# VinAIResearch/COMBAT

Hardware: AMD Instinct MI355X
Metric: images/sec per alternated generator+surrogate step, CIFAR-10 bs=128, 1/2/4/8 GPU (higher is better)
Workload: dtype bf16; 1 GPU; train_generator.py --dataset cifar10 --pc 0.5 --noise_rate 0.08: alternated PreActResNet18 surrogate + UNet generator step (Phase C + Phase G, both Nesterov-SGD updates), bs=128 per GPU, on-device augmentation on; per_gpu_batch=128, global_batch=128, parallelism=dp1 (RCCL all-reduce of netC grads in Phase C, netG grads in Phase G), losses_finite=True, deterministic=True

## Files before the change

### combat_amd/_lib.py

```python
from __future__ import annotations

import ctypes as C
import os

HERE = os.path.dirname(os.path.abspath(__file__))
LIB_PATH = os.environ.get("COMBAT_HIP_LIB") or os.path.join(HERE, "libcombat_hip.so")

c_i32, c_i64, c_f32, c_vp = C.c_int32, C.c_int64, C.c_float, C.c_void_p


class ConvArgs(C.Structure):

    _fields_ = [
        ("N", c_i32), ("H", c_i32), ("W", c_i32), ("C", c_i32),
        ("P", c_i32), ("Q", c_i32), ("K", c_i32),
        ("R", c_i32), ("S", c_i32), ("stride", c_i32), ("pad", c_i32),
        ("mode", c_i32),
        ("src", c_vp), ("wpack", c_vp), ("kpad", c_i32), ("rows_pad", c_i32), ("dst", c_vp),
        ("pro_scale", c_vp), ("pro_shift", c_vp), ("pro_group_stride", c_i32), ("pro_act", c_i32),
        ("pro_slope", c_f32),
        ("bias", c_vp), ("add_pre", c_vp), ("mask_x", c_vp), ("mask_scale", c_vp), ("mask_shift", c_vp),
        ("mask_activated", c_i32), ("mask_group_stride", c_i32), ("mask_slope", c_f32), ("mask_mul_scale", c_i32),
        ("add_post", c_vp), ("tanh_out", c_i32),
        ("stats_kind", c_i32), ("stats", c_vp), ("xh_mean", c_vp), ("xh_rstd", c_vp),
# ... 36 lines not shown

SIGNATURES = {
    "combat_version": (C.c_char_p, []),
    "combat_abi_version": (C.c_int, []),
    "combat_set_deterministic": (None, [C.c_int]),
    "combat_get_deterministic": (C.c_int, []),
    "combat_conv_gemm": (C.c_int, [C.POINTER(ConvArgs), c_vp]),
    "combat_conv_gemm_pair": (C.c_int, [C.POINTER(ConvArgs), C.POINTER(ConvArgs), c_vp]),
    "combat_conv_workspace_bytes": (c_i64, [C.POINTER(ConvArgs)]),
    "combat_conv_pick_tile": (C.c_int, [C.POINTER(ConvArgs)]),
    "combat_conv_stats_granule": (C.c_int, [C.c_int]),
    "combat_conv_stats_layout": (C.c_int, [C.POINTER(ConvArgs), C.POINTER(c_i32), C.POINTER(c_i32)]),
    "combat_conv_wgrad": (C.c_int, [C.POINTER(WgradArgs), c_vp]),
    "combat_conv_wgrad_workspace_bytes": (c_i64, [C.POINTER(WgradArgs)]),
    "combat_conv_wgrad_reduce": (C.c_int, [C.POINTER(WgradArgs), c_vp]),
    "combat_pack_weights": (C.c_int, [c_vp, c_i32, c_i32, c_i32, c_i32, c_i32, c_vp, c_i32, c_i32, c_vp, c_i32,
                                      c_i32, c_vp]),
    "combat_norm_finalize": (C.c_int, [c_vp, c_i32, c_i32, c_i32, c_f32, c_f32, c_vp, c_vp, c_vp, c_vp, c_vp, c_vp,
                                       c_vp, c_vp, c_f32, c_vp, c_vp, c_i64, c_vp]),
    "combat_norm_scratch_bytes": (c_i64, [c_i32, c_i32]),
    "combat_bn_eval_fold": (C.c_int, [c_vp, c_vp, c_vp, c_vp, c_f32, c_i32, c_vp, c_vp, c_vp]),
    "combat_pack_weights_batch": (C.c_int, [c_vp, c_i32, c_vp]),
    "combat_bn_eval_fold_batch": (C.c_int, [c_vp, c_i32, c_f32, c_vp]),
    "combat_group_stats": (C.c_int, [c_vp, c_i32, c_i32, c_i32, c_vp, c_vp]),
    "combat_norm_bwd_finalize": (C.c_int, [c_vp, c_i32, c_i32, c_i32, c_f32, c_vp, c_vp, c_vp, c_vp, c_vp, c_vp,
                                           c_vp, c_vp, c_vp, c_i64, c_vp]),
    "combat_norm_bwd_apply": (C.c_int, [c_vp, c_vp, c_vp, c_vp, c_i64, c_i32, c_i32, c_i32, c_vp, c_vp, c_vp, c_vp]),
    "combat_norm_act_fused": (C.c_int, [c_vp, c_vp, c_i32, c_i32, c_i64, c_i32, c_f32, c_f32, c_vp, c_vp, c_vp, c_vp, c_vp,
                                        c_vp, c_vp, c_vp, c_f32, c_vp, c_vp, c_i64, c_vp, c_vp]),
    "combat_norm_add_act_fused": (C.c_int, [c_vp, c_vp, c_i32, c_i32, c_i64, c_i32, c_f32, c_f32, c_vp, c_vp, c_vp, c_vp, c_vp,
# ... 114 lines not shown
```

### combat_amd/csrc/capi.cpp

```cpp
#include "combat_hip.h"

#include <hip/hip_runtime.h>

#include <atomic>
#include <cstdlib>
#include <mutex>
#include <unordered_map>

#define COMBAT_ABI_VERSION 20

extern "C" const char *combat_version(void) { return "combat_hip gfx950 abi17"; }
extern "C" int combat_abi_version(void) { return COMBAT_ABI_VERSION; }

static std::atomic<int> g_deterministic{-1};
bool combat_deterministic() {
    int v = g_deterministic.load(std::memory_order_relaxed);
    if (v < 0) {
        const char *e = getenv("COMBAT_DETERMINISTIC");
        v = e && e[0] == '1';
        g_deterministic.store(v, std::memory_order_relaxed);
    }
    return v != 0;
}
extern "C" void combat_set_deterministic(int on) { g_deterministic.store(on ? 1 : 0, std::memory_order_relaxed); }
// ... 19 lines not shown
```

### combat_amd/csrc/conv_common.hpp

```cpp
#pragma once
#include "common.hpp"
#include <type_traits>

int conv3x3_pick(const combat_conv_args *a);
int conv3x3_stats_layout(const combat_conv_args *a, int tile, int *rows, int *rows_per_image);
int conv3x3_launch(const combat_conv_args *a, int tile, hipStream_t st);
int conv3x3d_pick(const combat_conv_args *a);
int conv3x3d_stats_layout(const combat_conv_args *a, int tile, int *rows, int *rows_per_image);
int conv3x3d_launch(const combat_conv_args *a, int tile, hipStream_t st);
int conv_gather_dma_bn(const combat_conv_args *a);
bool conv_gather_dma_parity_split(const combat_conv_args *a);
bool conv_c8_ok(const combat_conv_args *a);
int conv_c8_launch(const combat_conv_args *a, hipStream_t st);
bool conv_k8_ok(const combat_conv_args *a);
int conv_k8_launch(const combat_conv_args *a, hipStream_t st);
int conv_gather_dma_launch(const combat_conv_args *a, hipStream_t st);
int conv_gather_dma_pair_launch(const combat_conv_args *a, const combat_conv_args *b, hipStream_t st);
long conv_gather_dma_workspace(const combat_conv_args *a);
int conv_wgrad3x3_try(const combat_wgrad_args *a, hipStream_t st);
int conv_wgrad3x3_dma_try(const combat_wgrad_args *a, hipStream_t st);
long conv_wgrad3x3_dma_workspace(const combat_wgrad_args *a);
int conv_wgrad3x3_dma_reduce(const combat_wgrad_args *a, hipStream_t st);

template <int BM, int BN, int WGM_ = 0>
struct TileCfg {
    static constexpr int WGM = WGM_ ? WGM_ : ((BN == 16) ? 4 : 2);
    static constexpr int WGN = 4 / WGM;
    static constexpr int WM = BM / WGM;
    static constexpr int WN = BN / WGN;
    static constexpr int FM = WM / 16;
    static constexpr int FN = WN / 16;
    static constexpr int A_ITERS = BM / 32;
    static constexpr int B_ITERS = (BN + 31) / 32;
    static constexpr int EPS = BN + 4;
    static constexpr int STAGE_BYTES = 2 * (BM + BN) * 128;
    static constexpr int EP_BYTES = BM * EPS * 4;
    static constexpr int SMEM = STAGE_BYTES > EP_BYTES ? STAGE_BYTES : EP_BYTES;
// ... 181 lines not shown
```

### combat_amd/csrc/conv_wgrad.hip

```cpp
#include "conv_common.hpp"
#include "plan.hpp"

namespace {

struct WgradParams {
    combat_wgrad_args a;
    int M, PQ, ntaps, tiles_k, tiles_c, split, pix_per_split;
    float *ws;
};

template <int BMC, int BNC>
struct WCfg {
    static constexpr int WGK = (BNC == 16) ? 4 : (BMC == 16 ? 1 : 2);
    static constexpr int WGC = 4 / WGK;
    static constexpr int WK = BMC / WGK;
    static constexpr int WC = BNC / WGC;
    static constexpr int FK = WK / 16;
    static constexpr int FC = WC / 16;
    static constexpr int SK = (BMC + 16) * 2;
    static constexpr int SC = (BNC + 16) * 2;
    static constexpr int CHK = BMC / 8;
    static constexpr int CHC = BNC / 8;
    static constexpr int ITK = (64 * CHK + 255) / 256;
    static constexpr int ITC = (64 * CHC + 255) / 256;
// ... 550 lines not shown
    if (a->R != a->S || (a->R != 1 && a->R != 3)) return COMBAT_EINVAL;
    if (a->stride != 1 && a->stride != 2) return COMBAT_EINVAL;
    if (a->c_real <= 0 || a->c_real > a->C || a->k_real <= 0 || a->k_real > a->K) return COMBAT_EINVAL;
    if ((a->pro_scale == nullptr) != (a->pro_shift == nullptr)) return COMBAT_EINVAL;
    if ((long)a->N * a->P * a->Q > 0x7fffffffL / 8) return COMBAT_EINVAL;
    return COMBAT_OK;
}

extern "C" int combat_conv_wgrad_reduce(const combat_wgrad_args *a, void *stream) {
    COMBAT_PLAN_HOOK(combat_conv_wgrad_reduce, a);
    if (validate_wgrad_args(a) != COMBAT_OK) return COMBAT_EINVAL;
    if (a->split < 0 || !a->defer_reduce) return COMBAT_OK;
    return conv_wgrad3x3_dma_reduce(a, as_stream(stream));
}

extern "C" int combat_conv_wgrad(const combat_wgrad_args *a, void *stream) {
    COMBAT_PLAN_HOOK(combat_conv_wgrad, a);
    if (validate_wgrad_args(a) != COMBAT_OK) return COMBAT_EINVAL;
    WgradParams p;
    p.a = *a;
    p.ws = nullptr;
    p.PQ = a->P * a->Q;
    p.M = (int)((long)a->N * p.PQ);
    p.ntaps = a->R * a->S;
    hipStream_t st = as_stream(stream);
    if (a->split >= 0) {
        int rc = conv_wgrad3x3_dma_try(a, st);
        if (rc <= 0) return rc;
    }
    if (a->reduce_first) {
// ... 15 lines not shown
```

### combat_amd/csrc/conv_wgrad3x3_dma.hip

```cpp
#include "conv_common.hpp"
#include <stdlib.h>

namespace {

typedef __attribute__((address_space(3))) void lds_void_t;
constexpr unsigned kOob = 0x40000000u;

struct W3dParams {
    combat_wgrad_args a;
    int TW, TH, TI, HWP, HH, HROWS, hpw, tw_shift, th_shift;
    int tiles_x, tiles_y, ntiles, tiles_k, tiles_c, split, per;
    unsigned x_bytes, dy_bytes;
    float *ws;
    const float *red_ws;
    float *red_dw;
    int red_base, red_tiles_c, red_split, red_k_real, red_c_real, red_pad;
    unsigned long long *stamps;
};

#ifdef COMBAT_STAMPS
static unsigned long long *g_stamps_wgrad_host = nullptr;
extern "C" int combat_debug_set_stamps_wgrad(void *p) { g_stamps_wgrad_host = (unsigned long long *)p; return 0; }
#define WCLK() __builtin_readcyclecounter()
#else
// ... 78 lines not shown
                const int row = (i * 2 + (wave & 1)) * 16 + (lane >> 4) * 4, col = (wave >> 1) * 16 + (lane & 15);
                const int tile_c = tile % tiles_c, tile_k = tile / tiles_c;
                const int n = tile_k * 64 + row, c = tile_c * 64 + col;
                if (c < c_real) {
#pragma unroll
                    for (int e = 0; e < 4; ++e)
                        if (n + e < k_real) dw[((size_t)(n + e) * 9 + tap) * c_real + c] += acc[u][e];
                }
            }
        }
        if (SL > 1) __syncthreads();
    }
}

template <int HPW, int NS, bool RED>
__device__ __forceinline__ void wgrad3x3_dma_body(const W3dParams &p) {
    extern __shared__ __attribute__((aligned(16))) unsigned char smem[];
    const combat_wgrad_args &a = p.a;
    const int tid = threadIdx.x, lane = tid & 63;
    const int wid = __builtin_amdgcn_readfirstlane(tid >> 6);
    const int wave_k = wid & 1, wave_c = wid >> 1;
    if (RED && p.red_ws) {
        reduce_slabs<512>(p.red_ws, p.red_dw, p.red_base, p.red_tiles_c, p.red_split, p.red_k_real, p.red_c_real, smem, blockIdx.x, gridDim.x);
        __syncthreads();
    }
    int bid = blockIdx.x;
    const int tile_c = bid % p.tiles_c; bid /= p.tiles_c;
    const int tile_k = bid % p.tiles_k;
    const int sp = bid / p.tiles_k;
    const int k0 = tile_k * 64, c0 = tile_c * 64;
    const int t_begin = sp * p.per;
    int t_end = t_begin + p.per;
    if (t_end > p.ntiles) t_end = p.ntiles;
    if (t_begin >= t_end) return;

    const int C = a.C, K = a.K, H = a.H, W = a.W;
    constexpr int XBYTES = HPW * 8192, DYBYTES = 64 * 128, DYBASE = NS * XBYTES;
    constexpr int NDMA = 1 + HPW;
    auto rsrc_words = [&](const void *ptr, unsigned bytes) __attribute__((always_inline)) {
        const unsigned long base = (unsigned long)ptr;
        u32x4_t w;
        w[0] = __builtin_amdgcn_readfirstlane((unsigned)base);
        w[1] = __builtin_amdgcn_readfirstlane((unsigned)(base >> 32) & 0xffffu);
        w[2] = __builtin_amdgcn_readfirstlane(bytes);
        w[3] = 0x00020000u;
        return w;
    };
    const u32x4_t xrs = rsrc_words(a.src, p.x_bytes), dyrs = rsrc_words(a.dy, p.dy_bytes);
    const unsigned lds0 = __builtin_amdgcn_readfirstlane((unsigned)(unsigned long)(lds_void_t *)smem) + wid * 1024;
#ifdef COMBAT_WGRAD_BUILTIN_DMA
    const __amdgpu_buffer_rsrc_t xrsrc = __builtin_amdgcn_make_buffer_rsrc(const_cast<void *>(a.src), 0, p.x_bytes, 0x00020000);
    const __amdgpu_buffer_rsrc_t dyrsrc = __builtin_amdgcn_make_buffer_rsrc(const_cast<void *>(a.dy), 0, p.dy_bytes, 0x00020000);
#define COMBAT_W3_DMA(rs_builtin, rs_words, lds_off, voff) \
    __builtin_amdgcn_raw_ptr_buffer_load_lds(rs_builtin, (lds_void_t *)(smem + (lds_off) + wid * 1024), 16, voff, 0, 0, 0)
#else
#define COMBAT_W3_DMA(rs_builtin, rs_words, lds_off, voff) \
    asm volatile("s_mov_b32 m0, %0\n\ts_nop 0\n\tbuffer_load_dwordx4 %1, %2, 0 offen lds" ::"s"(lds0_l + (unsigned)(lds_off)), "v"(voff), "s"(rs_words##_l) : "memory", "m0")
#endif

    int hdec[HPW], hrel[HPW];
#pragma unroll
    for (int j = 0; j < HPW; ++j) {
        const int row = (wid + 8 * j) * 8 + (lane >> 3), slot = lane & 7;
        const int hx = row % p.HWP, line = row / p.HWP;
        const int hy = line % p.HH, ti = line / p.HH;
        const int chunk = (((slot >> 1) ^ xkey(p.TW, line, hx)) << 1) | (slot & 1);
        hdec[j] = row < p.HROWS ? (hx | (hy << 8) | (ti << 16)) : -1;
// ... 172 lines not shown
#else
        (void)c0; (void)c1; (void)c2;
#endif
    };
    for (int i = 0; i < npatch; i += NS) {
        body(integral_constant<int, 0>{}, i);
        if (NS > 1 && i + 1 < npatch) body(integral_constant<int, 1 % NS>{}, i + 1);
        if (NS > 2 && i + 2 < npatch) body(integral_constant<int, 2 % NS>{}, i + 2);
    }
    }
    static_assert(NS == 2 || NS == 3, "the patch loop is unrolled for rings of two or three stages");
#ifdef COMBAT_STAMPS
    const unsigned long long c_loop1 = WCLK();
#endif

    if (p.ws) {
        float *slab = p.ws + (size_t)blockIdx.x * 9 * 4096;
#pragma unroll
        for (int tap = 0; tap < 9; ++tap)
#pragma unroll
            for (int i = 0; i < 2; ++i)
                *reinterpret_cast<f32x4_t *>(slab + tap * 4096 + ((i * 8 + wid) * 64 + lane) * 4) = acc[tap][i];
    } else {
        float *ep = reinterpret_cast<float *>(smem);
        constexpr int EPS = 68;
        const int fr = lane & 15;
#pragma unroll 1
        for (int tap = 0; tap < 9; ++tap) {
#pragma unroll
            for (int i = 0; i < 2; ++i) {
                const int col = wave_c * 16 + fr;
                const int row = (i * 2 + wave_k) * 16 + fq * 4;
// ... 4 lines not shown
                    case 2: v = acc[2][i]; break;
                    case 3: v = acc[3][i]; break;
                    case 4: v = acc[4][i]; break;
                    case 5: v = acc[5][i]; break;
                    case 6: v = acc[6][i]; break;
                    case 7: v = acc[7][i]; break;
                    default: v = acc[8][i]; break;
                }
#pragma unroll
                for (int e = 0; e < 4; ++e) ep[(row + e) * EPS + col] = v[e];
            }
            __syncthreads();
            for (int idx = tid; idx < 64 * 64; idx += 512) {
                const int row = idx >> 6, col = idx & 63;
                const int n = k0 + row, c = c0 + col;
                if (n < a.k_real && c < a.c_real) atomicAdd(a.dw + ((size_t)n * 9 + tap) * a.c_real + c, ep[row * EPS + col]);
            }
            __syncthreads();
        }
    }
#ifdef COMBAT_STAMPS
    if (lane == 0 && p.stamps) {
        unsigned long long *o = p.stamps + (blockIdx.x * 8 + wid) * 8;
        o[0] = ph[0]; o[1] = ph[1]; o[2] = ph[2]; o[3] = ph[3];
        o[4] = c_loop1 - c_loop0; o[5] = WCLK() - c_loop1; o[6] = c_loop0;
    }
#endif
}

__global__ __launch_bounds__(256) void wgrad3x3_reduce_kernel(const float *__restrict__ ws, float *__restrict__ dw,
                                                              int base, int tiles_c, int split, int k_real, int c_real) {
    const long e4 = (long)blockIdx.x * 256 + threadIdx.x;
    if (e4 >= (long)base * 9 * 1024) return;
    const int f4 = (int)(e4 & 1023), tap = (int)((e4 >> 10) % 9), tile = (int)(e4 / (9 * 1024));
    const int per = (split + gridDim.y - 1) / gridDim.y;
    const int s0 = blockIdx.y * per, s1 = s0 + per < split ? s0 + per : split;
    f32x4_t acc = {0.f, 0.f, 0.f, 0.f};
    const float *src = ws + ((size_t)tile * 9 + tap) * 4096 + f4 * 4;
    const size_t sstride = (size_t)base * 9 * 4096;
    int s = s0;
    for (; s + 4 <= s1; s += 4) {
        const f32x4_t v0 = *reinterpret_cast<const f32x4_t *>(src + (size_t)s * sstride);
        const f32x4_t v1 = *reinterpret_cast<const f32x4_t *>(src + (size_t)(s + 1) * sstride);
        const f32x4_t v2 = *reinterpret_cast<const f32x4_t *>(src + (size_t)(s + 2) * sstride);
        const f32x4_t v3 = *reinterpret_cast<const f32x4_t *>(src + (size_t)(s + 3) * sstride);
        acc += (v0 + v1) + (v2 + v3);
// ... 2 lines not shown
    const int i = f4 >> 9, wave = (f4 >> 6) & 7, lane = f4 & 63;
    const int row = (i * 2 + (wave & 1)) * 16 + (lane >> 4) * 4, col = (wave >> 1) * 16 + (lane & 15);
    const int tile_c = tile % tiles_c, tile_k = tile / tiles_c;
    const int n = tile_k * 64 + row, c = tile_c * 64 + col;
    if (c < c_real && s0 < s1) {
#pragma unroll
        for (int e = 0; e < 4; ++e) {
            if (n + e >= k_real) break;
            float *o = dw + ((size_t)(n + e) * 9 + tap) * c_real + c;
            if (gridDim.y == 1) *o += acc[e];
            else atomicAdd(o, acc[e]);
        }
    }
}

__global__ __launch_bounds__(256) void wgrad3x3_reduce_det_kernel(const float *__restrict__ ws, float *__restrict__ dw, int base,
                                                                  int tiles_c, int split, int k_real, int c_real) {
    __shared__ __attribute__((aligned(16))) unsigned char scratch[256 * 64];
    reduce_slabs<256>(ws, dw, base, tiles_c, split, k_real, c_real, scratch, blockIdx.x, gridDim.x);
}

template <int HPW, int NS, bool RED>
__global__ __launch_bounds__(512, 1) void conv_wgrad3x3_dma_kernel(const W3dParams p) { wgrad3x3_dma_body<HPW, NS, RED>(p); }

template <int HPW, int NS, bool RED>
int launch_w3d_red(const W3dParams &p, int blocks, hipStream_t st) {
    constexpr int stage = 8192 + HPW * 8192;
    constexpr int ep = 64 * 68 * 4;
    constexpr int smem = NS * stage > ep ? NS * stage : ep;
    auto kern = conv_wgrad3x3_dma_kernel<HPW, NS, RED>;
    static bool attr = false;
    if (!attr) {
        if (hipFuncSetAttribute(reinterpret_cast<const void *>(kern), hipFuncAttributeMaxDynamicSharedMemorySize, smem) != hipSuccess)
            return COMBAT_ELAUNCH;
        attr = true;
    }
    COMBAT_LAUNCH(kern, dim3(blocks), dim3(512), smem, st, p);
    CB_LAUNCH_CHECK();
    return COMBAT_OK;
}

template <int HPW, int NS>
int launch_w3d(const W3dParams &p, int blocks, hipStream_t st) {
    return p.red_ws ? launch_w3d_red<HPW, NS, true>(p, blocks, st) : launch_w3d_red<HPW, NS, false>(p, blocks, st);
}

bool w3d_geometry(const combat_wgrad_args *a, W3dParams &p, int &smem) {
    if (!(a->R == 3 && a->S == 3 && a->stride == 1 && a->pad == 1 && a->P == a->H && a->Q == a->W)) return false;
    if (a->pro_scale || a->pro_act) return false;
    if (a->C < 64 || (a->C & 63) || a->K < 64 || (a->K & 63) || a->c_real != a->C) return false;
    const int W = a->W, H = a->H;
    const int TW = W < 16 ? W : 16;
// ... 45 lines not shown

namespace {
bool w3d_plan(const combat_wgrad_args *a, W3dParams &p) {
    int smem;
    if (!w3d_geometry(a, p, smem)) return false;
    const int base = p.tiles_k * p.tiles_c;
    int split = pick_split(a, p, true);
    const bool use_ws = split > 1 && a->workspace && a->workspace_bytes >= (long)split * base * 9 * 4096 * 4;
    if (!use_ws) split = pick_split(a, p, false);
    p.ws = use_ws ? reinterpret_cast<float *>(a->workspace) : nullptr;
    p.per = (p.ntiles + split - 1) / split;
    p.split = (p.ntiles + p.per - 1) / p.per;
    return true;
}

int launch_reduce(const combat_wgrad_args *a, const W3dParams &p, hipStream_t st) {
    const int base = p.tiles_k * p.tiles_c;
    static const bool env_det = getenv("COMBAT_WGRAD_DET_REDUCE") != nullptr;
    const bool det = combat_deterministic();
    const bool atomics = !env_det && (!det || base >= 4);
    if (atomics) {
        const long e4 = (long)base * 9 * 1024;
        int groups = (int)(512 / ((e4 + 255) / 256));
        if (groups < 1 || det) groups = 1;
        if (groups > p.split) groups = p.split;
        COMBAT_LAUNCH(wgrad3x3_reduce_kernel, dim3((unsigned)((e4 + 255) / 256), groups), dim3(256), 0, st, p.ws, a->dw, base,
                           p.tiles_c, p.split, a->k_real, a->c_real);
    } else {
        COMBAT_LAUNCH(wgrad3x3_reduce_det_kernel, dim3(256), dim3(256), 0, st, (const float *)p.ws, a->dw, base, p.tiles_c, p.split,
                           a->k_real, a->c_real);
    }
    CB_LAUNCH_CHECK();
    return COMBAT_OK;
}

bool fill_reduce_first(const combat_wgrad_args *prev, W3dParams &p) {
    p.red_ws = nullptr;
    p.red_dw = nullptr;
    p.red_base = p.red_tiles_c = p.red_split = p.red_k_real = p.red_c_real = p.red_pad = 0;
    if (!prev) return true;
    W3dParams q;
    if (!w3d_plan(prev, q)) return true;
// ... 21 lines not shown
#endif
    const int blocks = p.tiles_k * p.tiles_c * p.split;
    int rc;
    if (p.hpw == 2) rc = launch_w3d<2, 3>(p, blocks, st);
    else if (p.hpw == 3) rc = launch_w3d<3, 2>(p, blocks, st);
    else rc = launch_w3d<4, 2>(p, blocks, st);
    if (rc != COMBAT_OK || !p.ws || a->defer_reduce) return rc;
    return launch_reduce(a, p, st);
}

int conv_wgrad3x3_dma_reduce(const combat_wgrad_args *a, hipStream_t st) {
    W3dParams p;
    if (!w3d_plan(a, p) || !p.ws) return COMBAT_OK;
    return launch_reduce(a, p, st);
}
```

### combat_amd/engine.py

```python
from __future__ import annotations

import ctypes
import os
from typing import Dict, List, Optional, Tuple

import torch

from . import ops
from ._lib import STATS_PER_WORKGROUP, TILE_D128x32, TILE_D128x64, TILE_S128x64, CombatHipError, ConvArgs, lib
from .nets import UNET_LAYERS
from .ops import Affine, PackedConv, bf16

BATCH_STATS_ROWS = 0 if os.environ.get("COMBAT_STATS_PER_WAVE") == "1" else STATS_PER_WORKGROUP

f32 = torch.float32


def _p(t):
    return None if t is None else t.data_ptr()


class Plan:

    serial = False
    serial_shortcuts = False
    default_aux_queues = 1
    flush_at_marks = False
    defer_reduces = os.environ.get("COMBAT_DEFER_REDUCE", "0") == "1"

    def __init__(self, name: str):
        self.name = name
        self.calls: List[Tuple] = []
        self._keep: List = []
        self.marks: Dict[int, int] = {}
        self.aux: Dict[int, int] = {}
        self.aux_queues = Plan.default_aux_queues
        self.wgrads: List[Tuple] = []
        self._ws = None
        self._cplan = None
        self._prog = None
        self.after: Dict[int, int] = {}
        self.pending_reduces: List[Tuple] = []
        self.chain: Dict[int, Tuple] = {}
# ... 134 lines not shown
            auxs = [_aux_stream(stream, k) for k in range(self.aux_queues)]
        used = set()
        awaited = set(self.after.values()) if auxs else set()
        done: Dict[int, torch.cuda.Event] = {}
        for ci, (cfunc, args, what) in enumerate(self.calls):
            if auxs and ci in self.after and self.after[ci] in done:
                (auxs[self.aux[ci]] if ci in self.aux else stream).wait_event(done[self.after[ci]])
            if prof is not None and cfunc is lib.combat_conv_gemm_pair:
                rc = 0
                for sub, arg in zip(what.split("+"), args):
                    e0, e1 = torch.cuda.Event(enable_timing=True), torch.cuda.Event(enable_timing=True)
                    e0.record(stream)
                    rc = rc or lib.combat_conv_gemm(arg, st)
                    e1.record(stream)
                    prof.append((self.name + "/" + sub, arg._obj, e0, e1))
            elif prof is not None and (cfunc is lib.combat_conv_gemm or cfunc is lib.combat_conv_wgrad or
                                       cfunc is lib.combat_conv_wgrad_reduce):
                e0, e1 = torch.cuda.Event(enable_timing=True), torch.cuda.Event(enable_timing=True)
                e0.record(stream)
                rc = cfunc(*args, st)
                e1.record(stream)
                prof.append((self.name + "/" + what, args[0]._obj, e0, e1))
            elif auxs and ci in self.aux:
                q = self.aux[ci]
                ev = torch.cuda.Event()
                ev.record(stream)
                auxs[q].wait_event(ev)
                rc = cfunc(*args, auxs[q].cuda_stream)
                used.add(q)
            else:
# ... 289 lines not shown

def balance_wgrads(plan: Plan, device) -> None:
    tail = int(os.environ.get("COMBAT_WGRAD_MAIN_TAIL", WGRAD_MAIN_TAIL))
    if tail <= 0 or Plan.serial:
        return
    aux_calls = [(ci, a) for ci, a in plan.wgrads if ci in plan.aux]
    ws = _wgrad_workspace(device, -1)
    plan._prog = None
    for ci, a in aux_calls[-tail:]:
        plan.aux.pop(ci, None)
        a.workspace, a.workspace_bytes = ws.data_ptr(), ws.numel()
        plan.hold(ws)


WGRAD_MAIN_TAIL = 0


_WGRAD_WS: Dict = {}


def _wgrad_workspace(device, queue: int = 0) -> torch.Tensor:
    key = (device, int(queue))
    ws = _WGRAD_WS.get(key)
    if ws is None:
        ws = torch.empty(48 << 20, dtype=torch.uint8, device=device)
        _WGRAD_WS[key] = ws
    return ws


def rec_act(plan: Plan, what: str, src, dst, aff: Affine):
# ... 488 lines not shown
                    tsc = slot.buf("g.b%d.tsc" % b, xin.shape)
                    rec_conv(P, "b%d.sc.dgrad" % b, d_out, tsc, blk.sc, 1)
            rec_wgrad(P, "b%d.c1.wgrad" % b, a0, dy1, blk.conv1, fp.grad_phys(pre + "conv1.weight"))
            self._dgrad_norm(P, slot, "g." + blk.bn1.prefix, dy1, dz1, blk.conv1, xin, st1, group_stride=0,
                             slope=0.0, gamma=blk.bn1.gamma, dgamma=fp.grad_phys(pre + "bn1.weight"),
                             dbeta=fp.grad_phys(pre + "bn1.bias"), add_pre=tsc, shortcut=fused)
            dxin = slot.buf("g.b%d.dx" % b, xin.shape)
            self._bwd_apply(P, slot, "g." + blk.bn1.prefix, dz1, xin, dxin, st1,
                            add=None if blk.sc is not None else d_out)
            d_out = dxin
            if b in (6, 4, 2):
                P.mark(fp.offsets[pre + "bn1.weight"][0])
        rec_wgrad(P, "stem.wgrad", self.input(slot), d_out, self.stem, fp.grad_phys("conv1.weight"), aux=False)
        P.mark(0)
        balance_wgrads(P, self.device)
        slot.plans[key] = P
        return P

    def two_loss_halves(self, slot: Slot):
        halves = getattr(slot, "two_loss_halves", None)
        if halves is None:
            assert slot.N % 2 == 0
            m = slot.N // 2
            h, x = self.head_bufs(slot), self.input(slot)
            gimg = slot.buf("g.img", (slot.N, slot.hw, slot.hw, 8))
            cells = ((h["loss"], h["correct"]),
                     (slot.buf("loss1", (1,), f32, zero=True), slot.buf("correct1", (2,), torch.int32, zero=True)))
            halves = []
            for k in range(2):
                s = Slot(slot.device, m, slot.hw)
# ... 225 lines not shown
                rec_conv(P, "b%d.c1.dgrad" % b, dy1, dxin, blk.conv1, 1, shortcut=fused, add_pre=other, mask_x=cur_in,
                         mask_activated=True)
                d_out = dxin
                if b in (6, 4, 2):
                    P.mark(fp.offsets[pre + "conv1.weight"][0])
            else:
                y0, st0 = slot.bufs["stem"], slot.norm[self.bn0.prefix]
                dz0 = G("stem.dz", y0)
                self._dgrad_norm(P, slot, "g." + self.bn0.prefix, dy1, dz0, blk.conv1, y0, st0, group_stride=0, slope=0.0,
                                 gamma=self.bn0.gamma, dgamma=fp.grad_phys("bn1.weight"), dbeta=fp.grad_phys("bn1.bias"),
                                 add_pre=other)
                dy0 = G("stem.dy", y0)
                self._bwd_apply(P, slot, "g." + self.bn0.prefix, dz0, y0, dy0, st0)
                rec_wgrad(P, "stem.wgrad", self.input(slot), dy0, self.stem, fp.grad_phys("conv1.weight"), aux=False)
        P.mark(0)
        slot.plans[key] = P
        return P

    def backward_eval_plan(self, slot: Slot, loss_weight: float, half_weights=None) -> Plan:
        if half_weights is not None:
            return self._two_loss_backward(slot, half_weights)
        key = "bwd.eval.%g" % loss_weight
        if key in slot.plans:
            return slot.plans[key]
        P = Plan("resnet." + key)
        n = slot.N
        d_out = self._head_grad(P, slot, loss_weight, False)
        for b in reversed(range(len(self.blocks))):
            blk = self.blocks[b]
            cur_in, a1 = self._block_in(slot, b), slot.bufs["b%d.a1" % b]
# ... 212 lines not shown
        P.mark(fp.offsets["conv3_0.weight"][0])
        d = through_norm("conv2_1", d, pc["conv2_1"], "conv2_0")
        d = through_norm("conv2_0", d, pc["conv2_0"], "conv1_1", add_pre=du1)
        d = through_norm("conv1_1", d, pc["conv1_1"], "conv1_0")
        d = through_norm("conv1_0", d, pc["conv1_0"], "conv0_1", add_pre=du0)
        t00 = t("conv0_0")
        lr_only = Affine(None, None, 0, True, self.LR)
        self._conv0_1_wgrad(P, slot, d)
        d00 = G("conv0_0.dx", t00)
        rec_conv(P, "conv0_1.dgrad", d, d00, pc["conv0_1"], 1, mask_x=t00, mask=Affine(None, None, 0, True, self.LR))
        P.add("db.conv0_0", lib.combat_colsum, d00.data_ptr(), d00.numel() // d00.shape[-1], d00.shape[-1],
              d00.shape[-1], fp.grad_phys("conv0_0.bias").data_ptr(), aux=True)
        rec_wgrad(P, "conv0_0.wgrad", self.input(slot), d00, pc["conv0_0"], fp.grad_phys("conv0_0.weight"), aux=False)
        P.mark(0)
        balance_wgrads(P, self.device)
        slot.plans["bwd"] = P
        return P


class CUnetEngine(UnetEngine):

    def __init__(self, module):
        self.num_classes = int(module.num_classes)
        super().__init__(module)

    def _w01(self) -> torch.Tensor:
        return self.fp._slice(self.fp.flat, "conv0_1.weight").view(self.nf, 3, 3, self.nf + self.num_classes)

    def _conv_operand(self, name: str, conv):
        if name != "conv0_1":
# ... 281 lines not shown
```

### include/combat_hip.h

```cpp
#ifndef COMBAT_HIP_H
#define COMBAT_HIP_H

#include <stdint.h>

#ifdef __cplusplus
extern "C" {
#endif

#define COMBAT_OK 0
#define COMBAT_EINVAL (-1)
#define COMBAT_ELAUNCH (-2)

const char *combat_version(void);
int combat_abi_version(void);

void combat_set_deterministic(int on);
int combat_get_deterministic(void);

typedef struct combat_conv_args {
    int32_t N, H, W, C;
    int32_t P, Q, K;
    int32_t R, S, stride, pad;
    int32_t mode;
    const void *src;
// ... 68 lines not shown
    const float *pro_scale, *pro_shift;
    int32_t pro_group_stride;
    int32_t pro_act;
    float pro_slope;
    int32_t split;
    void *workspace;
    int64_t workspace_bytes;
    int32_t defer_reduce;
    int32_t reserved;
    const struct combat_wgrad_args *reduce_first;
} combat_wgrad_args;

int combat_conv_wgrad(const combat_wgrad_args *a, void *stream);
int combat_conv_wgrad_reduce(const combat_wgrad_args *a, void *stream);
int64_t combat_conv_wgrad_workspace_bytes(const combat_wgrad_args *a);

int combat_pack_weights(const float *w, int32_t K, int32_t taps, int32_t c_real, int32_t C, int32_t dup_hilo,
                        void *wf, int32_t rows_pad_f, int32_t kpad_f,
                        void *wd, int32_t rows_pad_d, int32_t kpad_d, void *stream);
typedef struct combat_pack_desc {
    const float *w;
    void *wf, *wd;
    int32_t K, taps, c_real, C, dup_hilo, rows_pad_f, kpad_f, rows_pad_d, kpad_d;
    int32_t reserved;
    const float *row_scale;
} combat_pack_desc;
int combat_pack_weights_batch(const combat_pack_desc *descs, int32_t n, void *stream);

int combat_norm_finalize(const float *partials, int32_t groups, int32_t rows_per_group, int32_t C,
                         float count, float eps, const float *gamma, const float *beta,
// ... 198 lines not shown
```

Before: 32590 images/sec.

## Batch same-shape 3x3 weight-gradient convs into one grouped launch per stage

Adds a grouped weight-gradient kernel that runs up to four same-shape 3x3 wgrad problems in one launch, with the member selected by blockIdx.y, plus a grouped split-reduce kernel. A planner pass merges consecutive eligible wgrad calls on the same aux queue and stage into a single grouped call, on by default in 'stages' mode. The goal is to cut launch count and fill the GPU better when each wgrad alone is small, such as the ResNet18 blocks at bs=128. In exchange it needs a larger shared workspace, rewrites the plan indices, and may delay overlap between individual wgrads and other work.

Measured after the change: 33220 images/sec, median of 6. 1.9% higher.

```diff
diff --git a/combat_amd/_lib.py b/combat_amd/_lib.py
--- a/combat_amd/_lib.py
+++ b/combat_amd/_lib.py
@@ -74,6 +74,8 @@
     "combat_conv_wgrad": (C.c_int, [C.POINTER(WgradArgs), c_vp]),
     "combat_conv_wgrad_workspace_bytes": (c_i64, [C.POINTER(WgradArgs)]),
     "combat_conv_wgrad_reduce": (C.c_int, [C.POINTER(WgradArgs), c_vp]),
+    "combat_conv_wgrad_group": (C.c_int, [C.POINTER(C.POINTER(WgradArgs)), c_i32, c_vp, c_i64, c_vp]),
+    "combat_conv_wgrad_group_workspace_bytes": (c_i64, [C.POINTER(C.POINTER(WgradArgs)), c_i32]),
     "combat_pack_weights": (C.c_int, [c_vp, c_i32, c_i32, c_i32, c_i32, c_i32, c_vp, c_i32, c_i32, c_vp, c_i32,
                                       c_i32, c_vp]),
     "combat_norm_finalize": (C.c_int, [c_vp, c_i32, c_i32, c_i32, c_f32, c_f32, c_vp, c_vp, c_vp, c_vp, c_vp, c_vp,
diff --git a/combat_amd/csrc/capi.cpp b/combat_amd/csrc/capi.cpp
--- a/combat_amd/csrc/capi.cpp
+++ b/combat_amd/csrc/capi.cpp
@@ -7,7 +7,7 @@
 #include <mutex>
 #include <unordered_map>
 
-#define COMBAT_ABI_VERSION 20
+#define COMBAT_ABI_VERSION 21
 
 extern "C" const char *combat_version(void) { return "combat_hip gfx950 abi17"; }
 extern "C" int combat_abi_version(void) { return COMBAT_ABI_VERSION; }
diff --git a/combat_amd/csrc/conv_common.hpp b/combat_amd/csrc/conv_common.hpp
--- a/combat_amd/csrc/conv_common.hpp
+++ b/combat_amd/csrc/conv_common.hpp
@@ -21,6 +21,8 @@
 int conv_wgrad3x3_dma_try(const combat_wgrad_args *a, hipStream_t st);
 long conv_wgrad3x3_dma_workspace(const combat_wgrad_args *a);
 int conv_wgrad3x3_dma_reduce(const combat_wgrad_args *a, hipStream_t st);
+int conv_wgrad3x3_dma_group(const combat_wgrad_args *const *members, int n, void *workspace, long workspace_bytes, hipStream_t st);
+long conv_wgrad3x3_dma_group_workspace(const combat_wgrad_args *const *members, int n);
 
 template <int BM, int BN, int WGM_ = 0>
 struct TileCfg {
diff --git a/combat_amd/csrc/conv_wgrad.hip b/combat_amd/csrc/conv_wgrad.hip
--- a/combat_amd/csrc/conv_wgrad.hip
+++ b/combat_amd/csrc/conv_wgrad.hip
@@ -588,6 +588,23 @@
     return conv_wgrad3x3_dma_reduce(a, as_stream(stream));
 }
 
+extern "C" int64_t combat_conv_wgrad_group_workspace_bytes(const combat_wgrad_args *const *members, int32_t n) {
+    if (!members || n < 1) return COMBAT_EINVAL;
+    for (int i = 0; i < n; ++i)
+        if (validate_wgrad_args(members[i]) != COMBAT_OK) return COMBAT_EINVAL;
+    const long bytes = conv_wgrad3x3_dma_group_workspace(members, n);
+    return bytes < 0 ? COMBAT_EINVAL : bytes;
+}
+
+extern "C" int combat_conv_wgrad_group(const combat_wgrad_args *const *members, int32_t n, void *workspace, int64_t workspace_bytes,
+                                       void *stream) {
+    COMBAT_PLAN_HOOK(combat_conv_wgrad_group, members, n, workspace, workspace_bytes);
+    if (!members || n < 1) return COMBAT_EINVAL;
+    for (int i = 0; i < n; ++i)
+        if (validate_wgrad_args(members[i]) != COMBAT_OK) return COMBAT_EINVAL;
+    return conv_wgrad3x3_dma_group(members, n, workspace, (long)workspace_bytes, as_stream(stream));
+}
+
 extern "C" int combat_conv_wgrad(const combat_wgrad_args *a, void *stream) {
     COMBAT_PLAN_HOOK(combat_conv_wgrad, a);
     if (validate_wgrad_args(a) != COMBAT_OK) return COMBAT_EINVAL;
diff --git a/combat_amd/csrc/conv_wgrad3x3_dma.hip b/combat_amd/csrc/conv_wgrad3x3_dma.hip
--- a/combat_amd/csrc/conv_wgrad3x3_dma.hip
+++ b/combat_amd/csrc/conv_wgrad3x3_dma.hip
@@ -116,7 +116,8 @@
 }
 
 template <int HPW, int NS, bool RED>
-__device__ __forceinline__ void wgrad3x3_dma_body(const W3dParams &p) {
+__device__ __forceinline__ void wgrad3x3_dma_body(const W3dParams &p, const void *src_p, const void *dy_p, float *dw_p, float *ws_p,
+                                                  const int bid_in) {
     extern __shared__ __attribute__((aligned(16))) unsigned char smem[];
     const combat_wgrad_args &a = p.a;
     const int tid = threadIdx.x, lane = tid & 63;
@@ -126,7 +127,7 @@
         reduce_slabs<512>(p.red_ws, p.red_dw, p.red_base, p.red_tiles_c, p.red_split, p.red_k_real, p.red_c_real, smem, blockIdx.x, gridDim.x);
         __syncthreads();
     }
-    int bid = blockIdx.x;
+    int bid = bid_in;
     const int tile_c = bid % p.tiles_c; bid /= p.tiles_c;
     const int tile_k = bid % p.tiles_k;
     const int sp = bid / p.tiles_k;
@@ -148,11 +149,11 @@
         w[3] = 0x00020000u;
         return w;
     };
-    const u32x4_t xrs = rsrc_words(a.src, p.x_bytes), dyrs = rsrc_words(a.dy, p.dy_bytes);
+    const u32x4_t xrs = rsrc_words(src_p, p.x_bytes), dyrs = rsrc_words(dy_p, p.dy_bytes);
     const unsigned lds0 = __builtin_amdgcn_readfirstlane((unsigned)(unsigned long)(lds_void_t *)smem) + wid * 1024;
 #ifdef COMBAT_WGRAD_BUILTIN_DMA
-    const __amdgpu_buffer_rsrc_t xrsrc = __builtin_amdgcn_make_buffer_rsrc(const_cast<void *>(a.src), 0, p.x_bytes, 0x00020000);
-    const __amdgpu_buffer_rsrc_t dyrsrc = __builtin_amdgcn_make_buffer_rsrc(const_cast<void *>(a.dy), 0, p.dy_bytes, 0x00020000);
+    const __amdgpu_buffer_rsrc_t xrsrc = __builtin_amdgcn_make_buffer_rsrc(const_cast<void *>(src_p), 0, p.x_bytes, 0x00020000);
+    const __amdgpu_buffer_rsrc_t dyrsrc = __builtin_amdgcn_make_buffer_rsrc(const_cast<void *>(dy_p), 0, p.dy_bytes, 0x00020000);
 #define COMBAT_W3_DMA(rs_builtin, rs_words, lds_off, voff) \
     __builtin_amdgcn_raw_ptr_buffer_load_lds(rs_builtin, (lds_void_t *)(smem + (lds_off) + wid * 1024), 16, voff, 0, 0, 0)
 #else
@@ -355,8 +356,8 @@
     const unsigned long long c_loop1 = WCLK();
 #endif
 
-    if (p.ws) {
-        float *slab = p.ws + (size_t)blockIdx.x * 9 * 4096;
+    if (ws_p) {
+        float *slab = ws_p + (size_t)bid_in * 9 * 4096;
 #pragma unroll
         for (int tap = 0; tap < 9; ++tap)
 #pragma unroll
@@ -391,7 +392,7 @@
             for (int idx = tid; idx < 64 * 64; idx += 512) {
                 const int row = idx >> 6, col = idx & 63;
                 const int n = k0 + row, c = c0 + col;
-                if (n < a.k_real && c < a.c_real) atomicAdd(a.dw + ((size_t)n * 9 + tap) * a.c_real + c, ep[row * EPS + col]);
+                if (n < a.k_real && c < a.c_real) atomicAdd(dw_p + ((size_t)n * 9 + tap) * a.c_real + c, ep[row * EPS + col]);
             }
             __syncthreads();
         }
@@ -405,8 +406,8 @@
 #endif
 }
 
-__global__ __launch_bounds__(256) void wgrad3x3_reduce_kernel(const float *__restrict__ ws, float *__restrict__ dw,
-                                                              int base, int tiles_c, int split, int k_real, int c_real) {
+__device__ __forceinline__ void reduce_ranges(const float *__restrict__ ws, float *__restrict__ dw, int base, int tiles_c, int split,
+                                              int k_real, int c_real) {
     const long e4 = (long)blockIdx.x * 256 + threadIdx.x;
     if (e4 >= (long)base * 9 * 1024) return;
     const int f4 = (int)(e4 & 1023), tap = (int)((e4 >> 10) % 9), tile = (int)(e4 / (9 * 1024));
@@ -439,6 +440,39 @@
     }
 }
 
+__global__ __launch_bounds__(256) void wgrad3x3_reduce_kernel(const float *__restrict__ ws, float *__restrict__ dw,
+                                                              int base, int tiles_c, int split, int k_real, int c_real) {
+    reduce_ranges(ws, dw, base, tiles_c, split, k_real, c_real);
+}
+
+constexpr int kGroupMax = 4;
+struct W3dGroup {
+    const void *src[kGroupMax];
+    const void *dy[kGroupMax];
+    float *dw[kGroupMax];
+    float *ws[kGroupMax];
+};
+template <class T>
+__device__ __forceinline__ T pick_member(const T (&v)[kGroupMax], int m) {
+    T r = v[0];
+    if (m == 1) r = v[1];
+    if (m == 2) r = v[2];
+    if (m == 3) r = v[3];
+    return r;
+}
+
+__global__ __launch_bounds__(256) void wgrad3x3_reduce_group_kernel(const W3dGroup g, int base, int tiles_c, int split, int k_real,
+                                                                    int c_real) {
+    const int m = blockIdx.z;
+    reduce_ranges(pick_member(g.ws, m), pick_member(g.dw, m), base, tiles_c, split, k_real, c_real);
+}
+__global__ __launch_bounds__(256) void wgrad3x3_reduce_det_group_kernel(const W3dGroup g, int base, int tiles_c, int split, int k_real,
+                                                                        int c_real) {
+    __shared__ __attribute__((aligned(16))) unsigned char scratch[256 * 64];
+    const int m = blockIdx.y;
+    reduce_slabs<256>(pick_member(g.ws, m), pick_member(g.dw, m), base, tiles_c, split, k_real, c_real, scratch, blockIdx.x, gridDim.x);
+}
+
 __global__ __launch_bounds__(256) void wgrad3x3_reduce_det_kernel(const float *__restrict__ ws, float *__restrict__ dw, int base,
                                                                   int tiles_c, int split, int k_real, int c_real) {
     __shared__ __attribute__((aligned(16))) unsigned char scratch[256 * 64];
@@ -446,7 +480,16 @@
 }
 
 template <int HPW, int NS, bool RED>
-__global__ __launch_bounds__(512, 1) void conv_wgrad3x3_dma_kernel(const W3dParams p) { wgrad3x3_dma_body<HPW, NS, RED>(p); }
+__global__ __launch_bounds__(512, 1) void conv_wgrad3x3_dma_kernel(const W3dParams p) {
+    wgrad3x3_dma_body<HPW, NS, RED>(p, p.a.src, p.a.dy, p.a.dw, p.ws, blockIdx.x);
+}
+
+template <int HPW, int NS>
+__global__ __launch_bounds__(512, 1) void conv_wgrad3x3_dma_group_kernel(const W3dParams p, const W3dGroup g) {
+    const int m = blockIdx.y;
+    wgrad3x3_dma_body<HPW, NS, false>(p, pick_member(g.src, m), pick_member(g.dy, m), pick_member(g.dw, m), pick_member(g.ws, m),
+                                      blockIdx.x);
+}
 
 template <int HPW, int NS, bool RED>
 int launch_w3d_red(const W3dParams &p, int blocks, hipStream_t st) {
@@ -461,6 +504,23 @@
         attr = true;
     }
     COMBAT_LAUNCH(kern, dim3(blocks), dim3(512), smem, st, p);
+    CB_LAUNCH_CHECK();
+    return COMBAT_OK;
+}
+
+template <int HPW, int NS>
+int launch_w3d_group(const W3dParams &p, const W3dGroup &g, int blocks, int n, hipStream_t st) {
+    constexpr int stage = 8192 + HPW * 8192;
+    constexpr int ep = 64 * 68 * 4;
+    constexpr int smem = NS * stage > ep ? NS * stage : ep;
+    auto kern = conv_wgrad3x3_dma_group_kernel<HPW, NS>;
+    static bool attr = false;
+    if (!attr) {
+        if (hipFuncSetAttribute(reinterpret_cast<const void *>(kern), hipFuncAttributeMaxDynamicSharedMemorySize, smem) != hipSuccess)
+            return COMBAT_ELAUNCH;
+        attr = true;
+    }
+    COMBAT_LAUNCH(kern, dim3(blocks, n), dim3(512), smem, st, p, g);
     CB_LAUNCH_CHECK();
     return COMBAT_OK;
 }
@@ -536,18 +596,24 @@
     return true;
 }
 
+bool reduce_by_ranges(int base) {
+    static const bool env_det = getenv("COMBAT_WGRAD_DET_REDUCE") != nullptr;
+    return !env_det && (!combat_deterministic() || base >= 4);
+}
+int reduce_range_groups(int base, int split) {
+    const long e4 = (long)base * 9 * 1024;
+    int groups = (int)(512 / ((e4 + 255) / 256));
+    if (groups < 1 || combat_deterministic()) groups = 1;
+    if (groups > split) groups = split;
+    return groups;
+}
+
 int launch_reduce(const combat_wgrad_args *a, const W3dParams &p, hipStream_t st) {
     const int base = p.tiles_k * p.tiles_c;
-    static const bool env_det = getenv("COMBAT_WGRAD_DET_REDUCE") != nullptr;
-    const bool det = combat_deterministic();
-    const bool atomics = !env_det && (!det || base >= 4);
-    if (atomics) {
+    if (reduce_by_ranges(base)) {
         const long e4 = (long)base * 9 * 1024;
-        int groups = (int)(512 / ((e4 + 255) / 256));
-        if (groups < 1 || det) groups = 1;
-        if (groups > p.split) groups = p.split;
-        COMBAT_LAUNCH(wgrad3x3_reduce_kernel, dim3((unsigned)((e4 + 255) / 256), groups), dim3(256), 0, st, p.ws, a->dw, base,
-                           p.tiles_c, p.split, a->k_real, a->c_real);
+        COMBAT_LAUNCH(wgrad3x3_reduce_kernel, dim3((unsigned)((e4 + 255) / 256), reduce_range_groups(base, p.split)), dim3(256), 0, st, p.ws,
+                      a->dw, base, p.tiles_c, p.split, a->k_real, a->c_real);
     } else {
         COMBAT_LAUNCH(wgrad3x3_reduce_det_kernel, dim3(256), dim3(256), 0, st, (const float *)p.ws, a->dw, base, p.tiles_c, p.split,
                            a->k_real, a->c_real);
@@ -599,3 +665,71 @@
     if (!w3d_plan(a, p) || !p.ws) return COMBAT_OK;
     return launch_reduce(a, p, st);
 }
+
+namespace {
+bool same_problem_shape(const combat_wgrad_args *a, const combat_wgrad_args *b) {
+    return a->N == b->N && a->H == b->H && a->W == b->W && a->C == b->C && a->P == b->P && a->Q == b->Q && a->K == b->K && a->R == b->R &&
+           a->S == b->S && a->stride == b->stride && a->pad == b->pad && a->k_real == b->k_real && a->c_real == b->c_real &&
+           a->split == b->split;
+}
+
+long group_member_bytes(const combat_wgrad_args *const *m, int n) {
+    if (!m || n < 1 || n > kGroupMax) return -1;
+    for (int i = 0; i < n; ++i) {
+        const combat_wgrad_args *a = m[i];
+        if (!a || !a->src || !a->dy || !a->dw || a->split < 0 || a->reduce_first || a->defer_reduce) return -1;
+        if (!same_problem_shape(m[0], a)) return -1;
+        for (int j = 0; j < i; ++j)
+            if (m[j]->dw == a->dw) return -1;
+    }
+    W3dParams p;
+    int smem;
+    if (!w3d_geometry(m[0], p, smem)) return -1;
+    return conv_wgrad3x3_dma_workspace(m[0]);
+}
+}
+
+long conv_wgrad3x3_dma_group_workspace(const combat_wgrad_args *const *m, int n) {
+    const long one = group_member_bytes(m, n);
+    return one < 0 ? -1 : one * n;
+}
+
+int conv_wgrad3x3_dma_group(const combat_wgrad_args *const *m, int n, void *workspace, long workspace_bytes, hipStream_t st) {
+    const long one = group_member_bytes(m, n);
+    if (one < 0 || (one > 0 && (!workspace || workspace_bytes < one * n))) return COMBAT_EINVAL;
+    W3dParams p;
+    W3dGroup g = {};
+    for (int i = 0; i < n; ++i) {
+        combat_wgrad_args b = *m[i];
+        b.workspace = one > 0 ? static_cast<char *>(workspace) + (size_t)i * one : nullptr;
+        b.workspace_bytes = one;
+        W3dParams q;
+        if (!w3d_plan(&b, q)) return COMBAT_EINVAL;
+        if (combat_deterministic() && !q.ws && q.split > 1) return COMBAT_EINVAL;
+        if (i == 0) p = q;
+        else if (q.split != p.split || q.per != p.per || (q.ws == nullptr) != (p.ws == nullptr)) return COMBAT_EINVAL;
+        g.src[i] = b.src;
+        g.dy[i] = b.dy;
+        g.dw[i] = b.dw;
+        g.ws[i] = q.ws;
+    }
+    fill_reduce_first(nullptr, p);
+    p.stamps = nullptr;
+    const int blocks = p.tiles_k * p.tiles_c * p.split;
+    int rc;
+    if (p.hpw == 2) rc = launch_w3d_group<2, 3>(p, g, blocks, n, st);
+    else if (p.hpw == 3) rc = launch_w3d_group<3, 2>(p, g, blocks, n, st);
+    else rc = launch_w3d_group<4, 2>(p, g, blocks, n, st);
+    if (rc != COMBAT_OK || !p.ws) return rc;
+    const combat_wgrad_args *a = m[0];
+    const int base = p.tiles_k * p.tiles_c;
+    if (reduce_by_ranges(base)) {
+        const long e4 = (long)base * 9 * 1024;
+        COMBAT_LAUNCH(wgrad3x3_reduce_group_kernel, dim3((unsigned)((e4 + 255) / 256), reduce_range_groups(base, p.split), n), dim3(256), 0,
+                      st, g, base, p.tiles_c, p.split, a->k_real, a->c_real);
+    } else {
+        COMBAT_LAUNCH(wgrad3x3_reduce_det_group_kernel, dim3(256, n), dim3(256), 0, st, g, base, p.tiles_c, p.split, a->k_real, a->c_real);
+    }
+    CB_LAUNCH_CHECK();
+    return COMBAT_OK;
+}
diff --git a/combat_amd/engine.py b/combat_amd/engine.py
--- a/combat_amd/engine.py
+++ b/combat_amd/engine.py
@@ -27,6 +27,7 @@
     default_aux_queues = 1
     flush_at_marks = False
     defer_reduces = os.environ.get("COMBAT_DEFER_REDUCE", "0") == "1"
+    wgrad_groups = os.environ.get("COMBAT_WGRAD_GROUP", "stages")
 
     def __init__(self, name: str):
         self.name = name
@@ -191,6 +192,14 @@
                     rc = rc or lib.combat_conv_gemm(arg, st)
                     e1.record(stream)
                     prof.append((self.name + "/" + sub, arg._obj, e0, e1))
+            elif prof is not None and cfunc is lib.combat_conv_wgrad_group:
+                rc = 0
+                for sub, arg in zip(what.split("+"), args[0]):
+                    e0, e1 = torch.cuda.Event(enable_timing=True), torch.cuda.Event(enable_timing=True)
+                    e0.record(stream)
+                    rc = rc or lib.combat_conv_wgrad(arg, st)
+                    e1.record(stream)
+                    prof.append((self.name + "/" + sub, arg.contents, e0, e1))
             elif prof is not None and (cfunc is lib.combat_conv_gemm or cfunc is lib.combat_conv_wgrad or
                                        cfunc is lib.combat_conv_wgrad_reduce):
                 e0, e1 = torch.cuda.Event(enable_timing=True), torch.cuda.Event(enable_timing=True)
@@ -510,6 +519,78 @@
 
 
 WGRAD_MAIN_TAIL = 0
+
+_WGRAD_GROUP_WS: Dict = {}
+
+
+def _wgrad_group_workspace(device, queue: int, need: int) -> torch.Tensor:
+    key = (device, int(queue))
+    ws = _WGRAD_GROUP_WS.get(key)
+    if ws is None or ws.numel() < need:
+        ws = torch.empty(max(need, 1), dtype=torch.uint8, device=device)
+        _WGRAD_GROUP_WS[key] = ws
+    return ws
+
+
+def group_wgrads(plan: Plan, device) -> None:
+    mode = Plan.wgrad_groups
+    if mode not in ("tail", "pairs", "stages") or Plan.serial:
+        return
+    cap = 2 if mode == "pairs" else 4
+    marks = sorted(plan.marks)
+    stage = lambda ci: sum(1 for m in marks if m < ci)
+    args_of = {ci: a for ci, a in plan.wgrads}
+    linked = set(plan.after) | set(plan.after.values())
+    PP = ctypes.POINTER(ops.WgradArgs)
+
+    def query(members):
+        arr = (PP * len(members))(*[ctypes.pointer(a) for a in members])
+        return arr, int(lib.combat_conv_wgrad_group_workspace_bytes(arr, len(members)))
+
+    runs, run = [], []
+    for ci in sorted(plan.aux):
+        a = args_of.get(ci)
+        ok = a is not None and plan.calls[ci][0] is lib.combat_conv_wgrad and ci not in linked
+        if ok and run and len(run) < cap and plan.aux[run[-1]] == plan.aux[ci] and stage(run[0]) == stage(ci) and \
+                query([args_of[c] for c in run] + [a])[1] >= 0:
+            run.append(ci)
+            continue
+        if len(run) > 1:
+            runs.append(run)
+        run = [ci] if ok and query([a])[1] >= 0 else []
+    if len(run) > 1:
+        runs.append(run)
+    if mode == "tail":
+        runs = runs[-1:]
+    elif mode == "pairs":
+        runs = [r for r in runs if stage(r[0]) == stage(runs[-1][0])]
+    if not runs:
+        return
+    replaced, dropped = {}, set()
+    for r in runs:
+        arr, need = query([args_of[c] for c in r])
+        ws = _wgrad_group_workspace(device, plan.aux[r[-1]], need)
+        plan.hold(arr, ws)
+        replaced[r[-1]] = (lib.combat_conv_wgrad_group, (arr, len(r), ws.data_ptr(), ws.numel()), "+".join(plan.calls[c][2] for c in r))
+        dropped.update(r[:-1])
+        for c in r[:-1]:
+            args_of[c] = None
+    assert not (dropped & set(plan.marks)), "an all-reduce mark on a weight-gradient call"
+    new_index, calls = {}, []
+    last_of = {c: r[-1] for r in runs for c in r}
+    for ci, call in enumerate(plan.calls):
+        if ci in dropped:
+            continue
+        new_index[ci] = len(calls)
+        calls.append(replaced.get(ci, call))
+    at = lambda ci: new_index[last_of.get(ci, ci)]
+    plan.calls = calls
+    plan.marks = {at(ci): off for ci, off in plan.marks.items()}
+    plan.aux = {at(ci): q for ci, q in plan.aux.items() if ci not in dropped}
+    plan.after = {at(ci): at(dep) for ci, dep in plan.after.items()}
+    plan.wgrads = [(at(ci), a) for ci, a in plan.wgrads]
+    plan.pending_reduces = [(w, a, at(ci)) for w, a, ci in plan.pending_reduces]
+    plan._prog = None
 
 
 _WGRAD_WS: Dict = {}
@@ -1028,6 +1109,7 @@
         rec_wgrad(P, "stem.wgrad", self.input(slot), d_out, self.stem, fp.grad_phys("conv1.weight"), aux=False)
         P.mark(0)
         balance_wgrads(P, self.device)
+        group_wgrads(P, self.device)
         slot.plans[key] = P
         return P
 
@@ -1283,6 +1365,7 @@
                 self._bwd_apply(P, slot, "g." + self.bn0.prefix, dz0, y0, dy0, st0)
                 rec_wgrad(P, "stem.wgrad", self.input(slot), dy0, self.stem, fp.grad_phys("conv1.weight"), aux=False)
         P.mark(0)
+        group_wgrads(P, self.device)
         slot.plans[key] = P
         return P
 
@@ -1525,6 +1608,7 @@
         rec_wgrad(P, "conv0_0.wgrad", self.input(slot), d00, pc["conv0_0"], fp.grad_phys("conv0_0.weight"), aux=False)
         P.mark(0)
         balance_wgrads(P, self.device)
+        group_wgrads(P, self.device)
         slot.plans["bwd"] = P
         return P
 
diff --git a/include/combat_hip.h b/include/combat_hip.h
--- a/include/combat_hip.h
+++ b/include/combat_hip.h
@@ -106,6 +106,9 @@
 int combat_conv_wgrad(const combat_wgrad_args *a, void *stream);
 int combat_conv_wgrad_reduce(const combat_wgrad_args *a, void *stream);
 int64_t combat_conv_wgrad_workspace_bytes(const combat_wgrad_args *a);
+int combat_conv_wgrad_group(const combat_wgrad_args *const *members, int32_t n, void *workspace, int64_t workspace_bytes,
+                            void *stream);
+int64_t combat_conv_wgrad_group_workspace_bytes(const combat_wgrad_args *const *members, int32_t n);
 
 int combat_pack_weights(const float *w, int32_t K, int32_t taps, int32_t c_real, int32_t C, int32_t dup_hilo,
                         void *wf, int32_t rows_pad_f, int32_t kpad_f,
```
